# luanaruiz9/gated_gcrnns

Measured on AMD Instinct MI355X. Metric: sequences/sec (node), N=1000 K=5 T=32 F=64, higher is better.
Workload: dtype bf16

## Files before the change

gated_gcrnns_amd/_lib.py:

```python
import ctypes as C
import os

import torch

from . import build as _build

F32, F64, BF16 = 0, 1, 2

_c_i64 = C.c_int64
_c_p = C.c_void_p


class GcrnnError(RuntimeError):
    pass


def _load():
    path = os.environ.get('GCRNN_LIBPATH')
    if path:
        return _bind(C.CDLL(path))
    path = _build.LIBPATH
    if _build.needs_build() and os.path.exists(_build.HIPCC):
        _build.build(verbose=False)
    if not os.path.exists(path):
# ... 45 lines not shown
        'gcrnn_ell_assign_rows': (C.c_int, [_c_p, _c_p, _c_i64, _c_p, C.c_int, _c_i64, _c_p]),
        'gcrnn_fused_supported': (C.c_int, [_c_i64, _c_i64, _c_i64, _c_i64]),
        'gcrnn_fused_padded_nodes': (_c_i64, []),
        'gcrnn_fused_step_waves': (_c_i64, []),
        'gcrnn_fused_wgrad_waves': (_c_i64, []),
        'gcrnn_pack_seq_major': (C.c_int, [C.c_int, _c_p, _c_p, _c_i64, _c_i64, _c_i64, _c_i64, _c_i64, _c_p, _c_p]),
        'gcrnn_pack_seq_major_padded': (C.c_int, [_c_p, _c_p] + [_c_i64] * 6 + [_c_p]),
        'gcrnn_unpack_seq_major': (C.c_int, [C.c_int, _c_p, _c_p, _c_i64, _c_i64, _c_i64, _c_i64, _c_i64, _c_p, _c_p]),
        'gcrnn_fused_pack_weights': (C.c_int, [C.c_int, _c_p, _c_p, _c_p, _c_i64, _c_i64, _c_i64, _c_i64, _c_p]),
        'gcrnn_fused_forward_bf16': (C.c_int, [_c_p, _c_p, _c_p, _c_p, _c_p, _c_p, _c_p, _c_p, _c_p, _c_p, _c_p,
                                               _c_p, _c_p,
                                               _c_i64, _c_i64, _c_i64, _c_i64, _c_i64, _c_i64, _c_i64, _c_p, C.c_int, _c_p, C.c_double, _c_p, _c_p, _c_p, _c_p]),
        'gcrnn_fused_pack_weights_wide': (C.c_int, [C.c_int, _c_p, _c_p, _c_p, _c_i64, _c_i64, _c_i64, _c_i64, _c_i64, C.c_double, _c_p]),
        'gcrnn_fused_forward_wide_supported': (C.c_int, [_c_i64] * 7 + [C.c_double, C.c_int, C.c_int]),
        'gcrnn_fused_forward_wide_bf16': (C.c_int, [_c_p] * 10 + [_c_i64] * 7 + [_c_p, C.c_int, _c_p, _c_p, _c_p, _c_p]),
        'gcrnn_fused_backward_data_wide_supported': (C.c_int, [_c_i64] * 6 + [C.c_double, C.c_int, C.c_int]),
        'gcrnn_fused_backward_data_wide_bf16': (C.c_int, [_c_p] * 8 + [_c_i64] * 6 + [_c_p] * 7),
        'gcrnn_gate_readout_finish': (C.c_int, [_c_p, _c_i64, _c_p, _c_p, _c_p, _c_p, _c_i64, _c_p]),
        'gcrnn_fused_filter_output_wide_supported': (C.c_int, [_c_i64] * 7 + [C.c_double, C.c_int, C.c_int]),
        'gcrnn_fused_filter_output_wide_bf16': (C.c_int, [_c_p] * 7 + [_c_i64] * 7 + [_c_p, _c_p]),
        'gcrnn_fused_node_forward_wide_supported': (C.c_int, [_c_i64] * 6 + [C.c_double, C.c_int]),
        'gcrnn_fused_node_forward_wide_bf16': (C.c_int, [_c_p] * 11 + [_c_i64] * 6 + [_c_p, C.c_int, _c_p]),
        'gcrnn_fused_gate_pair_wide_supported': (C.c_int, [_c_i64] * 7 + [C.c_double, C.c_int, C.c_int]),
        'gcrnn_fused_gate_pair_prepass_wide_bf16': (C.c_int, [_c_p] * 12 + [_c_i64] * 7 + [_c_p, _c_p, _c_p, _c_p]),
        'gcrnn_fused_gate_pair_prepass_taps_wide_bf16': (C.c_int, [_c_p] * 7 + [_c_i64] + [_c_p] * 5 + [_c_i64] * 7 + [_c_p, _c_p, _c_p, _c_p]),
        'gcrnn_fused_inline_pack_supported': (C.c_int, [_c_i64, _c_i64, _c_i64, _c_i64, _c_i64, C.c_double]),
        'gcrnn_fused_seq_steps_per_launch': (_c_i64, [_c_i64] * 7 + [C.c_double, C.c_int, C.c_int, C.c_int]),
        'gcrnn_fused_filter_output_bf16': (C.c_int, [_c_p] * 11 + [_c_i64] * 7 + [C.c_double, C.c_int, _c_p]),
        'gcrnn_fused_node_forward_bf16': (C.c_int, [_c_p] * 15 + [_c_i64] * 6 + [_c_p, C.c_int, C.c_double, _c_p]),
        'gcrnn_fused_node_backward_data_bf16': (C.c_int, [_c_p] * 12 + [_c_i64] * 6 + [C.c_double, _c_p, C.c_int, _c_p]),
# ... 103 lines not shown
```

gated_gcrnns_amd/csrc/gcrnn_fused_seq32.h:

```cpp
#pragma once

#if defined(GCRNN_SEQ_STAMPS)
static __device__ unsigned long long gcrnn_seq32_stamps[256 * 96];
static __device__ __forceinline__ void gcrnn_stamp32_put(uint32_t lds_addr) {
  const unsigned long long tv = __builtin_amdgcn_s_memtime();
  asm volatile("ds_write_b64 %0, %1" ::"v"(lds_addr), "v"(tv) : "memory");
}
static __device__ __forceinline__ unsigned long long gcrnn_stamp32_get(uint32_t lds_addr) {
  unsigned long long tv;
  asm volatile("ds_read_b64 %0, %1\n\ts_waitcnt lgkmcnt(0)" : "=v"(tv) : "v"(lds_addr) : "memory");
  return tv;
}
#define GCRNN_STAMP32(slot)                                                                                   \
  do {                                                                                                        \
    if (wave == 0 && stamp_on && lane_now() == 0) gcrnn_stamp32_put((uint32_t)reinterpret_cast<uintptr_t>(smem) + M::FLAG_OFF + 8 * (slot)); \
  } while (0)
#define GCRNN_STAMP32_WAVE(slot0)                                                                             \
  do {                                                                                                        \
    if (stamp_on && lane_now() == 0) gcrnn_stamp32_put((uint32_t)reinterpret_cast<uintptr_t>(smem) + M::FLAG_OFF + 8 * ((slot0) + wave)); \
  } while (0)
#define GCRNN_STAMP32_FLUSH()                                                                                 \
  do {                                                                                                        \
    __syncthreads();                                                                                          \
    if (threadIdx.x < 96 && blockIdx.x < 256) gcrnn_seq32_stamps[blockIdx.x * 96 + threadIdx.x] = gcrnn_stamp32_get((uint32_t)reinterpret_cast<uintptr_t>(smem) + M::FLAG_OFF + 8 * threadIdx.x); \
// ... 63 lines not shown
  int hmod;
  const int32_t* flags;
  const float* gw;
  const uint4* tapf; float* taps_out; int ntaps;
  float* go;
  uint16_t* out1;
  const uint16_t* dh0_; int64_t dhstride;
  const uint16_t* hs0; int64_t hsstride;
  const float* gsc0; int64_t gscstride;
  float* gpart0; int64_t gpartstride;
  int final_raw;
  uint16_t* final_out; const uint16_t* final_h;
  const float* ng0; int64_t ngstride; int64_t nghalf;
  const float* r1a; const float* r1b;
  int stagger;
};

__device__ __forceinline__ int lane_now() {
  int ln;
  asm volatile("v_mbcnt_lo_u32_b32 %0, -1, 0\n\tv_mbcnt_hi_u32_b32 %0, -1, %0" : "=v"(ln));
  return ln;
}

#define GCRNN_HOP_ASM_WIDE32_STREAM(D)                                                             \
  do {                                                                                             \
    const int gwbeg = tbeg[0] >> 2, gwend = tend[STILES - 1] >> 2;                                 \
    if (gwbeg < gwend) {                                                                           \
      const int ls_ = lane_now(), r = ls_ & 15, q = ls_ >> 4;                                      \
      const uint32_t colb = lds_col + r * 8 + (q >> 1) * 4;        \
      const uint32_t qh_ = (uint32_t)(q & 1) << 4;                                                 \
// ... 22 lines not shown
  static_assert(16 * RS2 <= BIAS_OFF && FLAG_OFF + 768 <= WOFF, "LDS map");
  static size_t lds_bytes(int64_t entries, bool inline_pack, bool r1 = false) {
    const size_t need = (size_t)COL_OFF + (size_t)entries * 32 + GCRNN_HOP_COLUMN_PAD + NP * 4 + (r1 ? 2 * NP * 4 : 0) + (inline_pack ? (size_t)(32 * (XS > 0 ? XS : HS)) * NPCK * 2 : 0)
                        + PFS;
    return need <= 160 * 1024 ? need : 0;
  }
};

template <int K, int HS, int XS, int VAR, int MODE = 0, bool GATED = false, bool R1 = false, bool SPLIT = false>
__global__ __launch_bounds__(STHREADS) void fused_seq32_kernel(const Seq32Args a) {
  static_assert(!R1 || !SPLIT, "rank-1 graphs: every mode of the persistent form (the BPTT chain takes the adjoint plan: the factors swap)");
  static_assert(!SPLIT || ((MODE == 0 || MODE == 2) && !R1 && HS > 1), "split sequences: the (un-gated or time-gated) forward and the BPTT chain, with more than one chunk");
  constexpr bool ITEMS = (MODE == 1 || MODE == 3);
  constexpr bool SONLY = (MODE == 2 || MODE == 4);
  constexpr bool PKV = (VAR & 1) != 0, USERV = (VAR & 2) != 0 && (MODE == 0 || MODE == 4);
  static_assert(MODE == 0 || ((MODE >= 1 && MODE <= 4) && !GATED), "modes");
  static_assert(MODE < 3 || (!R1 && !SPLIT), "modes 3, 4: uniform-weight graphs, persistent form");
  using M = Seq32Map<K, HS, XS>;
  constexpr int KS = HS + XS;
  constexpr int F = 32 * HS, G = 32 * XS;
  constexpr int NCH = (MODE == 1) ? 2 * HS : HS;
  constexpr int PL = M::PL, WOFF = M::WOFF, WB = M::WB, COL_OFF = M::COL_OFF, RS2 = M::RS2;
  constexpr int NPCK = M::NPCK, NRND = NP / NPCK, NH = NCH * (K - 1), RPH = (NRND + NH - 1) / NH;
  constexpr int PKROWS = SONLY ? F : G;
  static_assert(STILES == 8 && GCRNN_HOP_ASM && K >= 2 && (SONLY ? XS == 0 : XS > 0), "generated hop stream: 8 tiles per wave; the chain's operand is the state alone");
  extern __shared__ __attribute__((aligned(16))) char smem[];
  const int entries = a.entries, B = a.B, N = a.N;

  const int tid = threadIdx.x, lane = tid & 63;
  const int wave = __builtin_amdgcn_readfirstlane(tid >> 6);
// ... 450 lines not shown
            lds_barrier();
            pack_drain(r0 + e);
          }
        }
#if !GCRNN_SEQ32_EP_FIRST
        if constexpr (SONLY && EPH > 0 && j <= EPH)
          ep_request(std::integral_constant<int, (j - 1) * STILES / (EPH > 0 ? EPH : 1)>{}, std::integral_constant<int, j * STILES / (EPH > 0 ? EPH : 1)>{});
#endif
        if (j < K - 1) lds_barrier();
        GCRNN_STAMP32(1 + chunk * 24 + 4 * (j - 1) + 4);
      };
      seq_static_for(hop, std::make_integer_sequence<int, K - 1>{});

      typedef __attribute__((__vector_size__(4 * sizeof(unsigned int)))) unsigned int u32x4_t;
      const int lane = lane_now(), q = lane >> 4, tl = wave * 64 + lane;
      auto request_next_operand = [&]() {
        if (ITEMS || !(last && more)) return;
        const int qo = lane_now() >> 4;
        int sw[STILES];
        slot_words(lane, sw);
        const __amdgpu_buffer_rsrc_t rsrc_hn = __builtin_amdgcn_make_buffer_rsrc(hout, 0, B * (NP * F * 2), 0x00020000);
#pragma unroll
        for (int s = 0; s < KS; ++s) {
          if (s == HS - 1) continue;
#pragma unroll
          for (int i = 0; i < STILES; ++i) {
            const int w = sw[i];
#ifdef GCRNN_SEQ32_EXPERIMENT_SKIP
            if ((GCRNN_SEQ32_EXPERIMENT_SKIP == 1) == (s < HS)) continue;
#endif
            if (s < HS)
              bfr[i][s] = __builtin_bit_cast(bf16x8, __builtin_amdgcn_raw_buffer_load_b128(rsrc_hn, (w >> 16) * (F * 2) + 16 * qo + 64 * s, b * (NP * F * 2), GCRNN_SEQ32_NT_XLOAD));
            else
              bfr[i][s] = __builtin_bit_cast(bf16x8, __builtin_amdgcn_raw_buffer_load_b128(rsrc_xn, (w >> 16) * (G * 2) + 16 * qo + 64 * (s - HS), b * (NP * G * 2), GCRNN_SEQ32_NT_XLOAD));
          }
        }
      };
      if (GCRNN_SEQ32_OPERAND_AT == 0) request_next_operand();
      if (ITEMS) GCRNN_STAMP32(1 + chunk * 24 + 19);
      float bs[2][4];
#pragma unroll
      for (int h = 0; h < 2; ++h)
#pragma unroll
        for (int e = 0; e < 4; ++e) bs[h][e] = (MODE >= 3 ? 1.f : (gin + gfo)) * lbias[chunk * 32 + q * 8 + h * 4 + e];
      u32x4_t pkd[STILES];
      int swe[STILES];
// ... 141 lines not shown
          if (lane == 0) gpart[(int64_t)b * (NCH * SWAVES) + chunk * SWAVES + wave] = part;
        }
      } else {
#pragma unroll
      for (int i = 0; i < STILES; ++i) {
        const int node = swe[i] >> 16;
        u32x4_t p{0u, 0u, 0u, 0u};
        if (node < N) {
          const f32x4 a0 = acc[i][0], a1 = acc[i][1];
          p[0] = pack2bf(fast_tanh(a0[0] + bs[0][0]), fast_tanh(a0[1] + bs[0][1]));
          p[1] = pack2bf(fast_tanh(a0[2] + bs[0][2]), fast_tanh(a0[3] + bs[0][3]));
          p[2] = pack2bf(fast_tanh(a1[0] + bs[1][0]), fast_tanh(a1[1] + bs[1][1]));
          p[3] = pack2bf(fast_tanh(a1[2] + bs[1][2]), fast_tanh(a1[3] + bs[1][3]));
        }
        pkd[i] = p;
        if (GCRNN_SEQ32_NT_STATE && last) __builtin_amdgcn_raw_buffer_store_b128(p, rsrc_o, node * (F * 2) + (chunk * 32 + q * 8) * 2, b * (NP * F * 2), GCRNN_SEQ32_NT_STATE);
        else __builtin_amdgcn_raw_buffer_store_b128(p, rsrc_o, node * (F * 2) + (chunk * 32 + q * 8) * 2, b * (NP * F * 2), 0);
        if (GCRNN_SEQ32_OPERAND_AT == 3 && last && more) {
          const __amdgpu_buffer_rsrc_t rsrc_hn = __builtin_amdgcn_make_buffer_rsrc(hout, 0, B * (NP * F * 2), 0x00020000);
#pragma unroll
          for (int s = 0; s < KS; ++s) {
            if (s == HS - 1) continue;
            if (s < HS)
              bfr[i][s] = __builtin_bit_cast(bf16x8, __builtin_amdgcn_raw_buffer_load_b128(rsrc_hn, node * (F * 2) + 16 * q + 64 * s, b * (NP * F * 2), 0));
            else
              bfr[i][s] = __builtin_bit_cast(bf16x8, __builtin_amdgcn_raw_buffer_load_b128(rsrc_xn, node * (G * 2) + 16 * q + 64 * (s - HS), b * (NP * G * 2), 0));
          }
        }
      }
      }
      GCRNN_STAMP32(1 + chunk * 24 + 17);
      if (!ITEMS && last) {
// ... 51 lines not shown
```

gated_gcrnns_amd/csrc/gcrnn_fused_seq32.hip:

```cpp
#include "gcrnn_fused_step.h"
#include "gcrnn_fused_seq32.h"

template <typename W>
__global__ void pack_weights_wide_kernel(const W* __restrict__ wA, const W* __restrict__ wB, uint16_t* __restrict__ out,
                                         int Fout, int F, int G, int Kin, int Kst, int K, float w) {
  const int KS = (F + G) / 32;
  const int64_t total = (int64_t)(Fout / 32) * K * 2 * KS * 64 * 8;
  const int64_t idx = (int64_t)blockIdx.x * blockDim.x + threadIdx.x;
  if (idx >= total) return;
  const int j = idx & 7, lane = (idx >> 3) & 63;
  int64_t rest = idx >> 9;
  const int s = rest % KS; rest /= KS;
  const int h = rest & 1; rest >>= 1;
  const int tap = rest % K;
  const int chunk = rest / K;
  const int m = lane & 15;
  const int f = chunk * 32 + 8 * (m >> 2) + 4 * h + (m & 3);
  const int feat = 32 * s + 8 * (lane >> 4) + j;
  float v = 0.f;
  if (feat < F) { if (tap < Kst) v = (float)wB[((int64_t)f * Kst + tap) * F + feat]; }
  else          { if (tap < Kin) v = (float)wA[((int64_t)f * Kin + tap) * G + (feat - F)]; }
  float sc = 1.f;
  for (int k = 0; k < tap; ++k) sc *= w;
  out[idx] = f2bf(v * sc);
// ... 158 lines not shown
    case 0: return seq32_launch_v<K, HS, XS, 0>(sa, lds, st);
    case 1: return seq32_launch_v<K, HS, XS, 1>(sa, lds, st);
    case 2: return seq32_launch_v<K, HS, XS, 2>(sa, lds, st);
    default: return seq32_launch_v<K, HS, XS, 3>(sa, lds, st);
  }
}

template <int K, int HS, int XS>
static int seq32_launch_pair(const Seq32Args& sa, bool inline_pack, hipStream_t st) {
  const size_t lds = seq32_lds<K, HS, XS>(sa.entries, inline_pack, sa.r1a != nullptr);
  if (!lds) return GCRNN_ERR_UNSUPPORTED;
  if (sa.r1a) return inline_pack ? seq32_launch_v<K, HS, XS, 1, 1, false, true>(sa, lds, st) : seq32_launch_v<K, HS, XS, 0, 1, false, true>(sa, lds, st);
  return inline_pack ? seq32_launch_v<K, HS, XS, 1, 1>(sa, lds, st) : seq32_launch_v<K, HS, XS, 0, 1>(sa, lds, st);
}

extern "C" int gcrnn_fused_forward_wide_bf16(const void* xs, const void* h0, void* hs, const void* wpack, const float* bias,
                                             const float* gi, const float* gf, const int32_t* tile_nodes, const int32_t* tile_off, const void* ell_col4, int64_t entries,
                                             int64_t B, int64_t T, int64_t N, int64_t F, int64_t G, int64_t K, void* Huser,
                                             int huser_last_only, const void* Xuser_inline, const float* rank1_a, const float* rank1_b,
                                             void* stream) {
  if (!xs || !h0 || !hs || !wpack || !tile_nodes || !tile_off || !ell_col4) return GCRNN_ERR_NULL_POINTER;
  if ((rank1_a == nullptr) != (rank1_b == nullptr)) return GCRNN_ERR_BAD_SHAPE;
  if ((gi == nullptr) != (gf == nullptr) || (gi && Xuser_inline)) return GCRNN_ERR_BAD_SHAPE;
  if (B <= 0 || T <= 0 || N <= 0 || N > NP || B > (1 << 24) || entries <= 0 || entries % 4) return GCRNN_ERR_BAD_SHAPE;
  if (B * (NP * (F > G ? F : G) * 2) > 2147483647LL || T * F * N > 2147483647LL) return GCRNN_ERR_BAD_SHAPE;
  if (Huser && (N % 8 != 0 || (reinterpret_cast<uintptr_t>(Huser) & 15))) return GCRNN_ERR_BAD_SHAPE;
  if (Xuser_inline && (N % 8 != 0 || (reinterpret_cast<uintptr_t>(Xuser_inline) & 15) || T * G * N > 2147483647LL)) return GCRNN_ERR_BAD_SHAPE;
  const int64_t xstep = B * NP * G, hstep = B * NP * F;
  Seq32Args sa{};
  sa.x0 = (const uint16_t*)xs; sa.xstride = xstep;
  sa.hfirst = (const uint16_t*)h0;
  sa.out0 = (uint16_t*)hs; sa.ostride = hstep;
  sa.wpack = (const uint4*)wpack; sa.bias = bias;
  sa.a1 = (const uint16_t*)Huser; sa.a1stride = F * N; sa.a1_last_only = huser_last_only ? 1 : 0;
  sa.ubstride = (int)((huser_last_only ? 1 : T) * F * N);
  sa.tile_nodes = tile_nodes; sa.tile_off = tile_off; sa.ell_col4 = (const uint2*)ell_col4;
  sa.entries = (int)entries; sa.B = (int)B; sa.N = (int)N;
  sa.nsteps = (int)T;
  sa.gi0 = gi; sa.gf0 = gf; sa.gstride = B;
  sa.r1a = rank1_a; sa.r1b = rank1_b;
  {
    const char* sg = getenv("GCRNN_SEQ32_STAGGER");
    sa.stagger = sg ? atoi(sg) : 0;
  }
  const bool inline_pack = Xuser_inline != nullptr && T > 2;
  if (inline_pack) {
    sa.pk_src0 = (const uint16_t*)Xuser_inline; sa.pksrc_stride = G * N;
    sa.pk_dst0 = const_cast<uint16_t*>(sa.x0); sa.pkdst_stride = xstep;
    sa.pk_stride = (int)(T * G * N);
  }
  hipStream_t st = as_stream(stream);
  const bool split = !rank1_a && !seq32_wanted(B) && seq32_split_wanted(B, F);
  const bool pack_split = Xuser_inline != nullptr && T > 1;
  if (split && pack_split && !inline_pack) {
    sa.pk_src0 = (const uint16_t*)Xuser_inline; sa.pksrc_stride = G * N;
    sa.pk_dst0 = const_cast<uint16_t*>(sa.x0); sa.pkdst_stride = xstep;
    sa.pk_stride = (int)(T * G * N);
  }
#define GCRNN_SEQ32_CASE(KK, HH, XX) if (K == KK && F == 32 * HH && G == 32 * XX) return seq32_launch<KK, HH, XX>(sa, split ? pack_split : inline_pack, st, split, T, N);
  GCRNN_SEQ32_CASE(5, 2, 2) GCRNN_SEQ32_CASE(4, 2, 2) GCRNN_SEQ32_CASE(3, 2, 2) GCRNN_SEQ32_CASE(2, 2, 2)
  GCRNN_SEQ32_CASE(5, 2, 1) GCRNN_SEQ32_CASE(4, 2, 1) GCRNN_SEQ32_CASE(3, 2, 1) GCRNN_SEQ32_CASE(2, 2, 1)
  GCRNN_SEQ32_CASE(5, 1, 1) GCRNN_SEQ32_CASE(4, 1, 1) GCRNN_SEQ32_CASE(3, 1, 1) GCRNN_SEQ32_CASE(2, 1, 1)
#undef GCRNN_SEQ32_CASE
  return GCRNN_ERR_UNSUPPORTED;
}


extern "C" int gcrnn_fused_gate_pair_wide_supported(int64_t B, int64_t T, int64_t N, int64_t F, int64_t G, int64_t K, int64_t entries,
                                                    double uniform_w, int img16, int with_pack) {
  if (uniform_w == 0.0 || !img16 || N <= 0 || N > NP || B <= 0 || T <= 0 || entries <= 0 || entries % 4) return 0;
  if (with_pack && (N % 8 || T * G * N > 2147483647LL)) return 0;
  if (B * T * (NP * (F > G ? F : G) * 2) > 2147483647LL) return 0;
  if (!seq32_wanted(B * T)) return 0;
  if (!seq32_lds_for(F, G, K, entries, with_pack != 0, (img16 & 2) != 0)) return 0;
  if (!with_pack) return 1;
  const int64_t first = B * T < gcrnn_persistent_grid() ? B * T : gcrnn_persistent_grid();
  return (int)((first + B - 1) / B);
}

// ... 177 lines not shown
```

gated_gcrnns_amd/ops.py:

```python
import ctypes as C
import os

import torch

from . import _lib
from ._lib import lib, check, dtype_code, GcrnnError


def _p(t):
    return C.c_void_p(t.data_ptr()) if t is not None else None


def _stream():
    return C.c_void_p(torch.cuda.current_stream().cuda_stream)


def require_device(*tensors):
    for t in tensors:
        if t is not None and not t.is_cuda:
            raise GcrnnError('gated_gcrnns_amd has no CPU path: move the module and its inputs to a ROCm '
                             'device (model.to("cuda"), x.cuda()); got a tensor on %s' % t.device)


def _pack_raw(x, perm=None):
# ... 296 lines not shown
    ok = fused_inline_pack_ok(plan, N, F, G, K)
    inline_arg = inline
    inline = (ok if inline is None else (ok and inline)) and X.data_ptr() % 16 == 0
    plan16 = fused_img16_plan(graph, False, None)
    wide = fused_wide_plan(graph, B, T, N, F, G, K, inline)
    if wide is None and plan16 is None:
        inl1 = inline_arg is not False and not os.environ.get('GCRNN_NO_INLINE_PACK') and X.data_ptr() % 16 == 0
        wide = fused_wide_plan(graph, B, T, N, F, G, K, inl1, rank1=True)
        if wide is None and inl1:
            inl1 = False
            wide = fused_wide_plan(graph, B, T, N, F, G, K, False, rank1=True)
        if wide is not None:
            inline = inl1
    if wide is not None:
        wpw = _fused_pack_weights_wide(wAc, wBc, wide['uniform_w'], st)
        for rep in range(reps + warm):
            if rep == warm:
                e0.record()
            _fused_forward_wide(wide, xs, h0s, hs, wAc, wBc, b32, B, T, N, F, G, K, H, False, Xc if inline else None, st, wpw=wpw)
        e1.record()
        torch.cuda.synchronize()
        per_step = 1e3 * e0.elapsed_time(e1) / (reps * T)
        return {'avg_us': per_step, 'launches': reps, 'inline_pack': bool(inline), 'steps_per_launch': T,
                'launch_avg_us': per_step * T, 'kernel': 'fused_seq32_kernel'}
    for rep in range(reps + 1):
        if rep == 1:
            torch.cuda.synchronize()
            e0.record()
        check(lib.gcrnn_fused_forward_bf16(_p(xs), _p(h0s), _p(hs), _p(wpack), _p(b32), None, None, *_fused_graph_args(plan16 or plan),
                                           B, T, N, F, G, K, _p(H) if H is not None else None, 2 if plan16 else 0, None, plan.get('uniform_w', 0.0),
                                           _p(Xc) if inline else None, None, None, st),
              'fused_forward')
    e1.record()
    torch.cuda.synchronize()
# ... 85 lines not shown
        return wpack
    return _cached_pack('taps32', (wA.detach(), wB.detach()), float(uniform_w), st, make)


def fused_wide_plan(graph, B, T, N, F, G, K, inline, rank1=False, gated=False):
    plan16 = fused_img16_plan(graph, False, None)
    if plan16 is None and rank1 and not os.environ.get('GCRNN_NO_IMG16'):
        plan16 = graph.fused_plan_rank1()
    if plan16 is None or F % 32 or G % 32:
        return None
    ok = lib.gcrnn_fused_forward_wide_supported(int(B), int(T), int(N), int(F), int(G), int(K), int(plan16['entries']),
                                                float(plan16.get('uniform_w', 0.0)), (3 if plan16.get('rank1') else 1) | (4 if gated else 0), 1 if inline else 0)
    return plan16 if ok else None


def _fused_forward_wide(plan16, xs, h0s, hs, wA, wB, b32, B, T, N, F, G, K, H, last_only, Xinline, st, wpw=None, gi=None, gf=None):
    if wpw is None:
        wpw = _fused_pack_weights_wide(wA.detach(), wB.detach(), plan16['uniform_w'], st)
    check(lib.gcrnn_fused_forward_wide_bf16(_p(xs), _p(h0s), _p(hs), _p(wpw), _p(b32), _p(gi), _p(gf), _p(plan16['tile_slots']), _p(plan16['tile_off']),
                                            _p(plan16['ell_col4']), plan16['entries'], B, T, N, F, G, K,
                                            _p(H) if H is not None else None, int(bool(last_only)), _p(Xinline) if Xinline is not None else None,
                                            _p(plan16.get('rank1_a')), _p(plan16.get('rank1_b')), st),
          'fused_forward_wide')


def fused_img16_plan(graph, gated, head):
    import os
    if os.environ.get('GCRNN_NO_IMG16'):
        return None
    return graph.fused_plan_img16()


def _fused_graph_args(plan):
# ... 11 lines not shown
    return s


def fused_inline_pack_ok(plan, N, F, G, K):
    if os.environ.get('GCRNN_NO_INLINE_PACK'):
        return False
    return bool(lib.gcrnn_fused_inline_pack_supported(int(N), int(F), int(G), int(K), int(plan['entries']), float(plan.get('uniform_w', 0.0))))


def fused_pad_taps(wA):
    F, G = wA.shape[0], wA.shape[3]
    Gp = fused_padded_inputs(F, G)
    return wA if Gp == G else torch.nn.functional.pad(wA, (0, Gp - G))


def fused_pack_inputs(X, h0, graph, overlap=False, first_only=False, channels=None):
    B, T, G, N = X.shape
    F = h0.shape[1]
    npad = graph.fused_plan()['npad']
    st = _stream()
    Xc, h0c = X.contiguous(), h0.contiguous()
    if channels is not None and channels != G:
        assert channels > G and not overlap and not first_only
        xs = torch.empty((T, B, npad, channels), dtype=torch.bfloat16, device=X.device)
        hs_all = torch.empty((T + 1, B, npad, F), dtype=torch.bfloat16, device=X.device)
        check(lib.gcrnn_pack_seq_major(_lib.BF16, _p(h0c), _p(hs_all), B, 1, F, N, npad, None, st), 'pack_seq')
        check(lib.gcrnn_pack_seq_major_padded(_p(Xc), _p(xs), B, T, G, channels, N, npad, st), 'pack_seq_padded')
        return xs, hs_all
    xs = torch.empty((T, B, npad, G), dtype=torch.bfloat16, device=X.device)
    hs_all = torch.empty((T + 1, B, npad, F), dtype=torch.bfloat16, device=X.device)
    check(lib.gcrnn_pack_seq_major(_lib.BF16, _p(h0c), _p(hs_all), B, 1, F, N, npad, None, st), 'pack_seq')
    if first_only:
        check(lib.gcrnn_pack_seq_major_steps(_p(Xc), _p(xs), B, T, G, N, npad, 0, min(2, T), 0, st), 'pack_seq_steps')
        return xs, hs_all
    if not overlap:
        check(lib.gcrnn_pack_seq_major(_lib.BF16, _p(Xc), _p(xs), B, T, G, N, npad, None, st), 'pack_seq')
        return xs, hs_all
    main = torch.cuda.current_stream(X.device)
    side = _side_stream(X.device)
    check(lib.gcrnn_pack_seq_major_steps(_p(Xc), _p(xs), B, T, G, N, npad, 0, 1, 0, st), 'pack_seq_steps')
    ready = torch.cuda.Event()
    ready.record(main)
    side.wait_event(ready)
    events = [None] * T
    sst = C.c_void_p(side.cuda_stream)
    blocks = int(os.environ.get('GCRNN_PACK_BLOCKS', torch.cuda.get_device_properties(X.device).multi_processor_count))
    for t in range(1, T):
        check(lib.gcrnn_pack_seq_major_steps(_p(Xc), _p(xs), B, T, G, N, npad, t, t + 1, blocks, sst), 'pack_seq_steps')
        ev = torch.cuda.Event()
        ev.record(side)
        events[t] = ev
    Xc.record_stream(side)
    xs.record_stream(side)
    return xs, hs_all, events


def fused_pack_inputs_gated(X, h0, graph, F, K):
    B, T, G, N = X.shape
    plan = graph.fused_plan()
    plan16 = fused_img16_plan(graph, True, None)
    steps = 0
    if plan16 is not None and X.dtype == torch.bfloat16 and X.is_contiguous() and X.data_ptr() % 16 == 0 and not os.environ.get('GCRNN_NO_INLINE_PACK'):
        _, steps = fused_gate_pair_plan(graph, B, T, N, F, G, K, True)
        if steps <= 0:
            steps = int(lib.gcrnn_fused_gate_prepass_lays_out(B, T, N, F, G, K, plan16['entries'], plan.get('uniform_w', 0.0), 1))
    if steps <= 0 or steps >= T:
        return fused_pack_inputs(X, h0, graph)
    npad = plan['npad']
    st = _stream()
    xs = torch.empty((T, B, npad, G), dtype=torch.bfloat16, device=X.device)
    hs_all = torch.empty((T + 1, B, npad, F), dtype=torch.bfloat16, device=X.device)
    check(lib.gcrnn_pack_seq_major(_lib.BF16, _p(h0.contiguous()), _p(hs_all), B, 1, F, N, npad, None, st), 'pack_seq')
    check(lib.gcrnn_pack_seq_major_steps(_p(X), _p(xs), B, T, G, N, npad, 0, steps, 0, st), 'pack_seq_steps')
    xs._pending_user = X
    xs._pending_steps = steps
    return xs, hs_all


def _pending_layout_for(xs, consumer_steps):
    x_user = getattr(xs, '_pending_user', None)
    if x_user is None:
        return None
    done = int(getattr(xs, '_pending_steps', 0))
    if consumer_steps > 0 and consumer_steps == done:
        return x_user
    T, B, npad, G = xs.shape
# ... 109 lines not shown
            Xz[:, :, :X.shape[2]] = X
            X = Xz
    elif packed is None:
        X, wA = fused_pad_operands(X, wA.detach())
    B, T, _, N = X.shape
    G = wA.shape[3]
    F = wA.shape[0]
    K = max(wA.shape[2], wB.shape[2])
    plan = graph.fused_plan()
    st = _stream()
    dev = X.device
    X = X.contiguous()
    h0 = h0.contiguous()
    events = None
    inline = False
    if packed is not None:
        xs, hs_all = packed
    elif gates is None and gate_values is None and X.data_ptr() % 16 == 0 and (
            fused_inline_pack_ok(plan, N, F, G, K) or (head is None and not os.environ.get('GCRNN_NO_INLINE_PACK')
                                                       and fused_wide_plan(graph, B, T, N, F, G, K, True, rank1=True) is not None)):
        xs, hs_all = fused_pack_inputs(X, h0, graph, first_only=True)
        inline = True
    elif gates is None and fused_overlap_ok(X):
        xs, hs_all, events = fused_pack_inputs(X, h0, graph, overlap=True)
    elif gates is not None and gate_values is None:
        xs, hs_all = fused_pack_inputs_gated(X, h0, graph, F, K)
    else:
        xs, hs_all = fused_pack_inputs(X, h0, graph)
    h0s, hs = hs_all[:1], hs_all[1:]
    gi = gf = None
    if gate_values is not None:
        gi, gf = (g.detach().float().contiguous() for g in gate_values)
        assert tuple(gi.shape) == (T, B) and tuple(gf.shape) == (T, B)
    elif gates is not None:
        hzero = fused_h0_zero_flag(h0)
        g = {}
        gp = {}
        for name in ('in', 'forget'):
            wA_g, wB_g, bias_g, lin_w, lin_b = gates[name]
            if wA_g.shape[3] != G:
                wA_g = torch.nn.functional.pad(wA_g.detach(), (0, G - wA_g.shape[3]))
            assert max(wA_g.shape[2], wB_g.shape[2]) == K and wA_g.shape[0] == F
            gp[name] = (wA_g, wB_g, bias_g, lin_w, lin_b)
# ... 20 lines not shown
        check(lib.gcrnn_fused_forward_bf16(_p(xs), _p(h0s), _p(hs), _p(wpack), _p(b32), _p(gi), _p(gf), *_fused_graph_args(plan16 or plan),
                                           B, T, N, F, G, K, None, 2 if plan16 else 0, evs, plan.get('uniform_w', 0.0), _p(X) if inline else None,
                                           _p(hw), _p(part), st), 'fused_forward')
        y = part.sum(dim=2)
        if head[1] is not None:
            y = y + head[1].detach().float().reshape(())
        return y.permute(1, 0, 2).unsqueeze(2).contiguous()
    wide = fused_wide_plan(graph, B, T, N, F, G, K, inline, rank1=True, gated=(gi is not None)) if (evs is None and head is None and not (gi is not None and inline)) else None
    if wide is not None:
        if native_out:
            assert not return_states
            _fused_forward_wide(wide, xs, h0s, hs, wA, wB, b32, B, T, N, F, G, K, None, False, X if inline else None, st, gi=gi, gf=gf)
            Hv = hs.permute(1, 0, 3, 2)[:, :, :, :N]
            return Hv[:, T - 1:] if last_only else Hv
        H = torch.empty((B, 1 if last_only else T, F, N), dtype=torch.bfloat16, device=dev)
        _fused_forward_wide(wide, xs, h0s, hs, wA, wB, b32, B, T, N, F, G, K, H if direct else None, last_only, X if inline else None, st, gi=gi, gf=gf)
        if not direct:
            src = hs[T - 1:] if last_only else hs
            check(lib.gcrnn_unpack_seq_major(_lib.BF16, _p(src), _p(H), B, 1 if last_only else T, F, N, plan['npad'], None, st), 'unpack_seq')
        if return_states:
            return hs_all, plan, H
        return H
    plan16 = fused_img16_plan(graph, gi is not None, None)
    wpack = _fused_pack_weights(wA, wB, st)
    if native_out:
        assert not return_states
        check(lib.gcrnn_fused_forward_bf16(_p(xs), _p(h0s), _p(hs), _p(wpack), _p(b32), _p(gi), _p(gf), *_fused_graph_args(plan16 or plan),
                                           B, T, N, F, G, K, None, (2 if plan16 else 0), evs,
                                           plan.get('uniform_w', 0.0), _p(X) if inline else None, None, None, st),
              'fused_forward')
        Hv = hs.permute(1, 0, 3, 2)[:, :, :, :N]
        return Hv[:, T - 1:] if last_only else Hv
    H = torch.empty((B, 1 if last_only else T, F, N), dtype=torch.bfloat16, device=dev)
    check(lib.gcrnn_fused_forward_bf16(_p(xs), _p(h0s), _p(hs), _p(wpack), _p(b32), _p(gi), _p(gf), *_fused_graph_args(plan16 or plan),
                                       B, T, N, F, G, K, _p(H) if direct else None, int(last_only) | (2 if plan16 else 0), evs,
                                       plan.get('uniform_w', 0.0), _p(X) if inline else None, None, None, st),
          'fused_forward')
# ... 2147 lines not shown
```

include/gcrnn.h:

```cpp
#ifndef GCRNN_H
#define GCRNN_H

#include <stdint.h>

#ifdef __cplusplus
extern "C" {
#endif

enum { GCRNN_F32 = 0, GCRNN_F64 = 1, GCRNN_BF16 = 2 };

enum {
  GCRNN_OK = 0,
  GCRNN_ERR_BAD_DTYPE = 1,
  GCRNN_ERR_BAD_SHAPE = 2,
  GCRNN_ERR_NULL_POINTER = 3,
  GCRNN_ERR_UNSUPPORTED = 4,
  GCRNN_ERR_LAUNCH = 5,
  GCRNN_ERR_WORKSPACE = 6
};

int gcrnn_version(void);
const char* gcrnn_status_string(int status);
const char* gcrnn_last_hip_error(void);

// ... 162 lines not shown
                             const void* Xuser_inline ,
                             const float* head_w ,
                             float* head_part ,
                             void* stream);

int gcrnn_fused_pack_weights_wide(int wdtype, const void* wA, const void* wB, void* wpack, int64_t Fout, int64_t F, int64_t G, int64_t Kin,
                                  int64_t Kst, double uniform_w, void* stream);
int gcrnn_fused_forward_wide_supported(int64_t B, int64_t T, int64_t N, int64_t F, int64_t G, int64_t K, int64_t entries, double uniform_w,
                                       int img16, int inline_pack);
int gcrnn_fused_forward_wide_bf16(const void* xs, const void* h0, void* hs, const void* wpack, const float* bias, const float* gi,
                                  const float* gf, const int32_t* tile_nodes, const int32_t* tile_off, const void* ell_col4, int64_t entries,
                                  int64_t B, int64_t T, int64_t N, int64_t F, int64_t G, int64_t K, void* Huser, int huser_last_only,
                                  const void* Xuser_inline,
                                  const float* rank1_a, const float* rank1_b ,
                                  void* stream);
int gcrnn_fused_gate_pair_wide_supported(int64_t B, int64_t T, int64_t N, int64_t F, int64_t G, int64_t K, int64_t entries, double uniform_w,
                                         int img16, int with_pack);
int gcrnn_fused_backward_data_wide_supported(int64_t B, int64_t T, int64_t N, int64_t F, int64_t K, int64_t entries, double uniform_w, int img16,
                                             int inline_pack);
int gcrnn_fused_backward_data_wide_bf16(const void* dHs, const void* hs, void* dpre, void* dh0, const void* wpackT, const int32_t* tile_nodes,
                                        const int32_t* tile_off, const void* ell_col4, int64_t entries, int64_t B, int64_t T, int64_t N,
                                        int64_t F, int64_t K, const float* gf, const void* h0s, float* dgf_parts, const void* dHuser_inline,
                                        const float* rank1_a, const float* rank1_b, void* stream);
int gcrnn_fused_filter_output_wide_supported(int64_t B, int64_t T, int64_t N, int64_t F, int64_t G, int64_t K, int64_t entries, double uniform_w,
                                             int img16, int with_pack );
int gcrnn_fused_filter_output_wide_bf16(const void* xs, const void* wpack, const float* bias, void* out, const int32_t* tile_nodes,
                                        const int32_t* tile_off, const void* ell_col4, int64_t entries, int64_t B, int64_t T, int64_t N,
                                        int64_t F, int64_t G, int64_t K,
                                        const void* x_user ,
                                        void* stream);
// ... 173 lines not shown
```

Before: 148,100.

## Route persistent forward hidden state through per-workgroup scratch instead of full state image

Adds a scratch-buffer variant of the persistent wide forward kernel. When no states are returned, the hidden state for non-final channel chunks is stored to and reloaded from a small per-workgroup scratch region, rather than written to the full T×B×NP×F sequence-major state image. The Python side also stops allocating the T-step state image on this lean path. This is meant to cut global memory traffic and allocation size. In exchange it adds a new kernel variant and a buffer sized by grid and channel count, and it falls back when the split form is selected.

```diff
diff --git a/gated_gcrnns_amd/_lib.py b/gated_gcrnns_amd/_lib.py
--- a/gated_gcrnns_amd/_lib.py
+++ b/gated_gcrnns_amd/_lib.py
@@ -83,6 +83,8 @@
         'gcrnn_fused_pack_weights_wide': (C.c_int, [C.c_int, _c_p, _c_p, _c_p, _c_i64, _c_i64, _c_i64, _c_i64, _c_i64, C.c_double, _c_p]),
         'gcrnn_fused_forward_wide_supported': (C.c_int, [_c_i64] * 7 + [C.c_double, C.c_int, C.c_int]),
         'gcrnn_fused_forward_wide_bf16': (C.c_int, [_c_p] * 10 + [_c_i64] * 7 + [_c_p, C.c_int, _c_p, _c_p, _c_p, _c_p]),
+        'gcrnn_fused_forward_wide_scratch_bytes': (_c_i64, [_c_i64, _c_i64, C.c_int]),
+        'gcrnn_fused_forward_wide_scratch_bf16': (C.c_int, [_c_p] * 3 + [_c_i64] + [_c_p] * 7 + [_c_i64] * 7 + [_c_p, C.c_int, _c_p, _c_p, _c_p, _c_p]),
         'gcrnn_fused_backward_data_wide_supported': (C.c_int, [_c_i64] * 6 + [C.c_double, C.c_int, C.c_int]),
         'gcrnn_fused_backward_data_wide_bf16': (C.c_int, [_c_p] * 8 + [_c_i64] * 6 + [_c_p] * 7),
         'gcrnn_gate_readout_finish': (C.c_int, [_c_p, _c_i64, _c_p, _c_p, _c_p, _c_p, _c_i64, _c_p]),
diff --git a/gated_gcrnns_amd/csrc/gcrnn_fused_seq32.h b/gated_gcrnns_amd/csrc/gcrnn_fused_seq32.h
--- a/gated_gcrnns_amd/csrc/gcrnn_fused_seq32.h
+++ b/gated_gcrnns_amd/csrc/gcrnn_fused_seq32.h
@@ -101,6 +101,7 @@
   const float* ng0; int64_t ngstride; int64_t nghalf;
   const float* r1a; const float* r1b;
   int stagger;
+  uint16_t* scr;
 };
 
 __device__ __forceinline__ int lane_now() {
@@ -153,6 +154,9 @@
   constexpr bool ITEMS = (MODE == 1 || MODE == 3);
   constexpr bool SONLY = (MODE == 2 || MODE == 4);
   constexpr bool PKV = (VAR & 1) != 0, USERV = (VAR & 2) != 0 && (MODE == 0 || MODE == 4);
+  constexpr bool SCRV = (VAR & 4) != 0;
+  static_assert(!SCRV || (MODE == 0 && !SPLIT && (VAR & 2) != 0), "state scratch: the persistent forward with the user-layout output");
+  constexpr int SCR_CH = NP * 64;
   static_assert(MODE == 0 || ((MODE >= 1 && MODE <= 4) && !GATED), "modes");
   static_assert(MODE < 3 || (!R1 && !SPLIT), "modes 3, 4: uniform-weight graphs, persistent form");
   using M = Seq32Map<K, HS, XS>;
@@ -633,12 +637,16 @@
 
       typedef __attribute__((__vector_size__(4 * sizeof(unsigned int)))) unsigned int u32x4_t;
       const int lane = lane_now(), q = lane >> 4, tl = wave * 64 + lane;
+      auto scratch_rsrc = [&]() {
+        return __builtin_amdgcn_make_buffer_rsrc(SCRV ? a.scr + (int64_t)blockIdx.x * ((HS - 1) * (SCR_CH / 2)) : nullptr, 0, SCRV ? (HS - 1) * SCR_CH : 0, 0x00020000);
+      };
       auto request_next_operand = [&]() {
         if (ITEMS || !(last && more)) return;
         const int qo = lane_now() >> 4;
         int sw[STILES];
         slot_words(lane, sw);
-        const __amdgpu_buffer_rsrc_t rsrc_hn = __builtin_amdgcn_make_buffer_rsrc(hout, 0, B * (NP * F * 2), 0x00020000);
+        const __amdgpu_buffer_rsrc_t rsrc_hn = __builtin_amdgcn_make_buffer_rsrc(SCRV ? nullptr : hout, 0, SCRV ? 0 : B * (NP * F * 2), 0x00020000);
+        [[maybe_unused]] const __amdgpu_buffer_rsrc_t rsrc_sn = scratch_rsrc();
 #pragma unroll
         for (int s = 0; s < KS; ++s) {
           if (s == HS - 1) continue;
@@ -648,7 +656,9 @@
 #ifdef GCRNN_SEQ32_EXPERIMENT_SKIP
             if ((GCRNN_SEQ32_EXPERIMENT_SKIP == 1) == (s < HS)) continue;
 #endif
-            if (s < HS)
+            if (SCRV && s < HS)
+              bfr[i][s] = __builtin_bit_cast(bf16x8, __builtin_amdgcn_raw_buffer_load_b128(rsrc_sn, (lane_now() & 15) * 64 + 16 * qo, s * SCR_CH + (wave * STILES + i) * 1024, 16));
+            else if (s < HS)
               bfr[i][s] = __builtin_bit_cast(bf16x8, __builtin_amdgcn_raw_buffer_load_b128(rsrc_hn, (w >> 16) * (F * 2) + 16 * qo + 64 * s, b * (NP * F * 2), GCRNN_SEQ32_NT_XLOAD));
             else
               bfr[i][s] = __builtin_bit_cast(bf16x8, __builtin_amdgcn_raw_buffer_load_b128(rsrc_xn, (w >> 16) * (G * 2) + 16 * qo + 64 * (s - HS), b * (NP * G * 2), GCRNN_SEQ32_NT_XLOAD));
@@ -820,8 +830,12 @@
           p[3] = pack2bf(fast_tanh(a1[2] + bs[1][2]), fast_tanh(a1[3] + bs[1][3]));
         }
         pkd[i] = p;
+        if constexpr (SCRV) {
+          if (!last) __builtin_amdgcn_raw_buffer_store_b128(p, scratch_rsrc(), (lane & 15) * 64 + 16 * q, chunk * SCR_CH + (wave * STILES + i) * 1024, 0);
+        } else
         if (GCRNN_SEQ32_NT_STATE && last) __builtin_amdgcn_raw_buffer_store_b128(p, rsrc_o, node * (F * 2) + (chunk * 32 + q * 8) * 2, b * (NP * F * 2), GCRNN_SEQ32_NT_STATE);
         else __builtin_amdgcn_raw_buffer_store_b128(p, rsrc_o, node * (F * 2) + (chunk * 32 + q * 8) * 2, b * (NP * F * 2), 0);
+        static_assert(!SCRV || GCRNN_SEQ32_OPERAND_AT != 3, "state scratch: the per-tile request form reads the state image");
         if (GCRNN_SEQ32_OPERAND_AT == 3 && last && more) {
           const __amdgpu_buffer_rsrc_t rsrc_hn = __builtin_amdgcn_make_buffer_rsrc(hout, 0, B * (NP * F * 2), 0x00020000);
 #pragma unroll
diff --git a/gated_gcrnns_amd/csrc/gcrnn_fused_seq32.hip b/gated_gcrnns_amd/csrc/gcrnn_fused_seq32.hip
--- a/gated_gcrnns_amd/csrc/gcrnn_fused_seq32.hip
+++ b/gated_gcrnns_amd/csrc/gcrnn_fused_seq32.hip
@@ -196,23 +196,47 @@
   return inline_pack ? seq32_launch_v<K, HS, XS, 1, 1>(sa, lds, st) : seq32_launch_v<K, HS, XS, 0, 1>(sa, lds, st);
 }
 
-extern "C" int gcrnn_fused_forward_wide_bf16(const void* xs, const void* h0, void* hs, const void* wpack, const float* bias,
-                                             const float* gi, const float* gf, const int32_t* tile_nodes, const int32_t* tile_off, const void* ell_col4, int64_t entries,
-                                             int64_t B, int64_t T, int64_t N, int64_t F, int64_t G, int64_t K, void* Huser,
-                                             int huser_last_only, const void* Xuser_inline, const float* rank1_a, const float* rank1_b,
-                                             void* stream) {
-  if (!xs || !h0 || !hs || !wpack || !tile_nodes || !tile_off || !ell_col4) return GCRNN_ERR_NULL_POINTER;
+int gcrnn_seq32s_forward(const Seq32Args& sa, int K, int HS, int XS, bool inline_pack, size_t lds, hipStream_t st);
+
+static int64_t seq32_scratch_need(int64_t B, int64_t F) {
+  const int64_t wgs = B < gcrnn_persistent_grid() ? B : gcrnn_persistent_grid();
+  return wgs * (F / 32 - 1) * (int64_t)NP * 64;
+}
+
+extern "C" int64_t gcrnn_fused_forward_wide_scratch_bytes(int64_t B, int64_t F, int rank1) {
+  if (B <= 0 || F <= 0 || F % 32) return -1;
+  const char* sw = getenv("GCRNN_SEQ32_STATE_SCRATCH");
+  if (sw && sw[0] == '0') return -1;
+  const char* p32 = getenv("GCRNN_SEQ32P");
+  if (p32 && p32[0] != '0') return -1;
+  if (!rank1 && !seq32_wanted(B) && seq32_split_wanted(B, F)) return -1;
+  return seq32_scratch_need(B, F);
+}
+
+static int forward_wide_impl(const void* xs, const void* h0, void* hs, void* scratch, int64_t scratch_bytes, bool no_image, const void* wpack, const float* bias,
+                             const float* gi, const float* gf, const int32_t* tile_nodes, const int32_t* tile_off, const void* ell_col4, int64_t entries,
+                             int64_t B, int64_t T, int64_t N, int64_t F, int64_t G, int64_t K, void* Huser,
+                             int huser_last_only, const void* Xuser_inline, const float* rank1_a, const float* rank1_b,
+                             void* stream) {
+  if (!xs || !h0 || (!no_image && !hs) || !wpack || !tile_nodes || !tile_off || !ell_col4) return GCRNN_ERR_NULL_POINTER;
+  if (no_image && !Huser) return GCRNN_ERR_NULL_POINTER;
   if ((rank1_a == nullptr) != (rank1_b == nullptr)) return GCRNN_ERR_BAD_SHAPE;
   if ((gi == nullptr) != (gf == nullptr) || (gi && Xuser_inline)) return GCRNN_ERR_BAD_SHAPE;
   if (B <= 0 || T <= 0 || N <= 0 || N > NP || B > (1 << 24) || entries <= 0 || entries % 4) return GCRNN_ERR_BAD_SHAPE;
   if (B * (NP * (F > G ? F : G) * 2) > 2147483647LL || T * F * N > 2147483647LL) return GCRNN_ERR_BAD_SHAPE;
   if (Huser && (N % 8 != 0 || (reinterpret_cast<uintptr_t>(Huser) & 15))) return GCRNN_ERR_BAD_SHAPE;
   if (Xuser_inline && (N % 8 != 0 || (reinterpret_cast<uintptr_t>(Xuser_inline) & 15) || T * G * N > 2147483647LL)) return GCRNN_ERR_BAD_SHAPE;
+  if (no_image) {
+    if (F % 32 || F < 32) return GCRNN_ERR_UNSUPPORTED;
+    const int64_t need = seq32_scratch_need(B, F);
+    if (scratch_bytes < need || (need > 0 && (!scratch || (reinterpret_cast<uintptr_t>(scratch) & 15)))) return GCRNN_ERR_BAD_SHAPE;
+  }
   const int64_t xstep = B * NP * G, hstep = B * NP * F;
   Seq32Args sa{};
   sa.x0 = (const uint16_t*)xs; sa.xstride = xstep;
   sa.hfirst = (const uint16_t*)h0;
-  sa.out0 = (uint16_t*)hs; sa.ostride = hstep;
+  sa.out0 = no_image ? nullptr : (uint16_t*)hs; sa.ostride = hstep;
+  sa.scr = no_image ? (uint16_t*)scratch : nullptr;
   sa.wpack = (const uint4*)wpack; sa.bias = bias;
   sa.a1 = (const uint16_t*)Huser; sa.a1stride = F * N; sa.a1_last_only = huser_last_only ? 1 : 0;
   sa.ubstride = (int)((huser_last_only ? 1 : T) * F * N);
@@ -233,6 +257,19 @@
   }
   hipStream_t st = as_stream(stream);
   const bool split = !rank1_a && !seq32_wanted(B) && seq32_split_wanted(B, F);
+  if (no_image) {
+    if (split) return GCRNN_ERR_UNSUPPORTED;
+#define GCRNN_SEQ32_CASE(KK, HH, XX) \
+    if (K == KK && F == 32 * HH && G == 32 * XX) { \
+      const size_t lds = seq32_lds<KK, HH, XX>(sa.entries, inline_pack, sa.r1a != nullptr); \
+      return lds ? gcrnn_seq32s_forward(sa, KK, HH, XX, inline_pack, lds, st) : GCRNN_ERR_UNSUPPORTED; \
+    }
+    GCRNN_SEQ32_CASE(5, 2, 2) GCRNN_SEQ32_CASE(4, 2, 2) GCRNN_SEQ32_CASE(3, 2, 2) GCRNN_SEQ32_CASE(2, 2, 2)
+    GCRNN_SEQ32_CASE(5, 2, 1) GCRNN_SEQ32_CASE(4, 2, 1) GCRNN_SEQ32_CASE(3, 2, 1) GCRNN_SEQ32_CASE(2, 2, 1)
+    GCRNN_SEQ32_CASE(5, 1, 1) GCRNN_SEQ32_CASE(4, 1, 1) GCRNN_SEQ32_CASE(3, 1, 1) GCRNN_SEQ32_CASE(2, 1, 1)
+#undef GCRNN_SEQ32_CASE
+    return GCRNN_ERR_UNSUPPORTED;
+  }
   const bool pack_split = Xuser_inline != nullptr && T > 1;
   if (split && pack_split && !inline_pack) {
     sa.pk_src0 = (const uint16_t*)Xuser_inline; sa.pksrc_stride = G * N;
@@ -245,6 +282,24 @@
   GCRNN_SEQ32_CASE(5, 1, 1) GCRNN_SEQ32_CASE(4, 1, 1) GCRNN_SEQ32_CASE(3, 1, 1) GCRNN_SEQ32_CASE(2, 1, 1)
 #undef GCRNN_SEQ32_CASE
   return GCRNN_ERR_UNSUPPORTED;
+}
+
+extern "C" int gcrnn_fused_forward_wide_bf16(const void* xs, const void* h0, void* hs, const void* wpack, const float* bias,
+                                             const float* gi, const float* gf, const int32_t* tile_nodes, const int32_t* tile_off, const void* ell_col4, int64_t entries,
+                                             int64_t B, int64_t T, int64_t N, int64_t F, int64_t G, int64_t K, void* Huser,
+                                             int huser_last_only, const void* Xuser_inline, const float* rank1_a, const float* rank1_b,
+                                             void* stream) {
+  return forward_wide_impl(xs, h0, hs, nullptr, 0, false, wpack, bias, gi, gf, tile_nodes, tile_off, ell_col4, entries, B, T, N, F, G, K, Huser,
+                           huser_last_only, Xuser_inline, rank1_a, rank1_b, stream);
+}
+
+extern "C" int gcrnn_fused_forward_wide_scratch_bf16(const void* xs, const void* h0, void* scratch, int64_t scratch_bytes, const void* wpack, const float* bias,
+                                                     const float* gi, const float* gf, const int32_t* tile_nodes, const int32_t* tile_off, const void* ell_col4,
+                                                     int64_t entries, int64_t B, int64_t T, int64_t N, int64_t F, int64_t G, int64_t K, void* Huser,
+                                                     int huser_last_only, const void* Xuser_inline, const float* rank1_a, const float* rank1_b,
+                                                     void* stream) {
+  return forward_wide_impl(xs, h0, nullptr, scratch, scratch_bytes, true, wpack, bias, gi, gf, tile_nodes, tile_off, ell_col4, entries, B, T, N, F, G, K, Huser,
+                           huser_last_only, Xuser_inline, rank1_a, rank1_b, stream);
 }
 
 
diff --git a/gated_gcrnns_amd/csrc/gcrnn_fused_seq32s.hip b/gated_gcrnns_amd/csrc/gcrnn_fused_seq32s.hip
--- /dev/null
+++ b/gated_gcrnns_amd/csrc/gcrnn_fused_seq32s.hip
@@ -0,0 +1,35 @@
+#include "gcrnn_fused_step.h"
+#define GCRNN_SEQ32_STAMP_READER_NAME gcrnn_debug_read_seq32s_stamps
+#include "gcrnn_fused_seq32.h"
+
+template <int K, int HS, int XS, int VAR, bool GATED, bool R1>
+static int seq32s_launch_v(const Seq32Args& sa, size_t lds, hipStream_t st) {
+  static_assert((VAR & 6) == 6, "state scratch: with the user-layout output");
+  auto sk = fused_seq32_kernel<K, HS, XS, VAR, 0, GATED, R1>;
+  if (hipFuncSetAttribute(reinterpret_cast<const void*>(sk), hipFuncAttributeMaxDynamicSharedMemorySize, (int)lds) != hipSuccess)
+    return GCRNN_ERR_LAUNCH;
+  GCRNN_PRE_LAUNCH();
+  sk<<<(unsigned)(sa.B < gcrnn_persistent_grid() ? sa.B : gcrnn_persistent_grid()), STHREADS, lds, st>>>(sa);
+  GCRNN_CHECK_LAUNCH();
+  return GCRNN_OK;
+}
+
+template <int K, int HS, int XS>
+static int seq32s_launch(const Seq32Args& sa, bool inline_pack, size_t lds, hipStream_t st) {
+  if (!sa.a1 || (HS > 1 && !sa.scr)) return GCRNN_ERR_NULL_POINTER;
+  if (sa.gi0) {
+    if (inline_pack) return GCRNN_ERR_BAD_SHAPE;
+    return sa.r1a ? seq32s_launch_v<K, HS, XS, 6, true, true>(sa, lds, st) : seq32s_launch_v<K, HS, XS, 6, true, false>(sa, lds, st);
+  }
+  if (sa.r1a) return inline_pack ? seq32s_launch_v<K, HS, XS, 7, false, true>(sa, lds, st) : seq32s_launch_v<K, HS, XS, 6, false, true>(sa, lds, st);
+  return inline_pack ? seq32s_launch_v<K, HS, XS, 7, false, false>(sa, lds, st) : seq32s_launch_v<K, HS, XS, 6, false, false>(sa, lds, st);
+}
+
+int gcrnn_seq32s_forward(const Seq32Args& sa, int K, int HS, int XS, bool inline_pack, size_t lds, hipStream_t st) {
+#define GCRNN_SEQ32S_CASE(KK, HH, XX) if (K == KK && HS == HH && XS == XX) return seq32s_launch<KK, HH, XX>(sa, inline_pack, lds, st);
+  GCRNN_SEQ32S_CASE(5, 2, 2) GCRNN_SEQ32S_CASE(4, 2, 2) GCRNN_SEQ32S_CASE(3, 2, 2) GCRNN_SEQ32S_CASE(2, 2, 2)
+  GCRNN_SEQ32S_CASE(5, 2, 1) GCRNN_SEQ32S_CASE(4, 2, 1) GCRNN_SEQ32S_CASE(3, 2, 1) GCRNN_SEQ32S_CASE(2, 2, 1)
+  GCRNN_SEQ32S_CASE(5, 1, 1) GCRNN_SEQ32S_CASE(4, 1, 1) GCRNN_SEQ32S_CASE(3, 1, 1) GCRNN_SEQ32S_CASE(2, 1, 1)
+#undef GCRNN_SEQ32S_CASE
+  return GCRNN_ERR_UNSUPPORTED;
+}
diff --git a/gated_gcrnns_amd/ops.py b/gated_gcrnns_amd/ops.py
--- a/gated_gcrnns_amd/ops.py
+++ b/gated_gcrnns_amd/ops.py
@@ -334,10 +334,11 @@
             inline = inl1
     if wide is not None:
         wpw = _fused_pack_weights_wide(wAc, wBc, wide['uniform_w'], st)
+        scr = fused_state_scratch(wide, B, F, dev) if H is not None else None
         for rep in range(reps + warm):
             if rep == warm:
                 e0.record()
-            _fused_forward_wide(wide, xs, h0s, hs, wAc, wBc, b32, B, T, N, F, G, K, H, False, Xc if inline else None, st, wpw=wpw)
+            _fused_forward_wide(wide, xs, h0s, hs, wAc, wBc, b32, B, T, N, F, G, K, H, False, Xc if inline else None, st, wpw=wpw, scratch=scr)
         e1.record()
         torch.cuda.synchronize()
         per_step = 1e3 * e0.elapsed_time(e1) / (reps * T)
@@ -453,9 +454,24 @@
     return plan16 if ok else None
 
 
-def _fused_forward_wide(plan16, xs, h0s, hs, wA, wB, b32, B, T, N, F, G, K, H, last_only, Xinline, st, wpw=None, gi=None, gf=None):
+def fused_state_scratch(plan16, B, F, dev):
+    need = int(lib.gcrnn_fused_forward_wide_scratch_bytes(int(B), int(F), 1 if plan16.get('rank1') else 0))
+    if need < 0:
+        return None
+    return torch.empty((need,), dtype=torch.uint8, device=dev)
+
+
+def _fused_forward_wide(plan16, xs, h0s, hs, wA, wB, b32, B, T, N, F, G, K, H, last_only, Xinline, st, wpw=None, gi=None, gf=None, scratch=None):
     if wpw is None:
         wpw = _fused_pack_weights_wide(wA.detach(), wB.detach(), plan16['uniform_w'], st)
+    if scratch is not None:
+        assert H is not None
+        check(lib.gcrnn_fused_forward_wide_scratch_bf16(_p(xs), _p(h0s), _p(scratch), int(scratch.numel()), _p(wpw), _p(b32), _p(gi), _p(gf), _p(plan16['tile_slots']),
+                                                        _p(plan16['tile_off']), _p(plan16['ell_col4']), plan16['entries'], B, T, N, F, G, K,
+                                                        _p(H), int(bool(last_only)), _p(Xinline) if Xinline is not None else None,
+                                                        _p(plan16.get('rank1_a')), _p(plan16.get('rank1_b')), st),
+              'fused_forward_wide_scratch')
+        return
     check(lib.gcrnn_fused_forward_wide_bf16(_p(xs), _p(h0s), _p(hs), _p(wpw), _p(b32), _p(gi), _p(gf), _p(plan16['tile_slots']), _p(plan16['tile_off']),
                                             _p(plan16['ell_col4']), plan16['entries'], B, T, N, F, G, K,
                                             _p(H) if H is not None else None, int(bool(last_only)), _p(Xinline) if Xinline is not None else None,
@@ -497,21 +513,22 @@
     return wA if Gp == G else torch.nn.functional.pad(wA, (0, Gp - G))
 
 
-def fused_pack_inputs(X, h0, graph, overlap=False, first_only=False, channels=None):
+def fused_pack_inputs(X, h0, graph, overlap=False, first_only=False, channels=None, states=True):
     B, T, G, N = X.shape
     F = h0.shape[1]
     npad = graph.fused_plan()['npad']
     st = _stream()
+    TS = T if states else 0
     Xc, h0c = X.contiguous(), h0.contiguous()
     if channels is not None and channels != G:
         assert channels > G and not overlap and not first_only
         xs = torch.empty((T, B, npad, channels), dtype=torch.bfloat16, device=X.device)
-        hs_all = torch.empty((T + 1, B, npad, F), dtype=torch.bfloat16, device=X.device)
+        hs_all = torch.empty((TS + 1, B, npad, F), dtype=torch.bfloat16, device=X.device)
         check(lib.gcrnn_pack_seq_major(_lib.BF16, _p(h0c), _p(hs_all), B, 1, F, N, npad, None, st), 'pack_seq')
         check(lib.gcrnn_pack_seq_major_padded(_p(Xc), _p(xs), B, T, G, channels, N, npad, st), 'pack_seq_padded')
         return xs, hs_all
     xs = torch.empty((T, B, npad, G), dtype=torch.bfloat16, device=X.device)
-    hs_all = torch.empty((T + 1, B, npad, F), dtype=torch.bfloat16, device=X.device)
+    hs_all = torch.empty((TS + 1, B, npad, F), dtype=torch.bfloat16, device=X.device)
     check(lib.gcrnn_pack_seq_major(_lib.BF16, _p(h0c), _p(hs_all), B, 1, F, N, npad, None, st), 'pack_seq')
     if first_only:
         check(lib.gcrnn_pack_seq_major_steps(_p(Xc), _p(xs), B, T, G, N, npad, 0, min(2, T), 0, st), 'pack_seq_steps')
@@ -538,7 +555,7 @@
     return xs, hs_all, events
 
 
-def fused_pack_inputs_gated(X, h0, graph, F, K):
+def fused_pack_inputs_gated(X, h0, graph, F, K, states=True):
     B, T, G, N = X.shape
     plan = graph.fused_plan()
     plan16 = fused_img16_plan(graph, True, None)
@@ -548,11 +565,11 @@
         if steps <= 0:
             steps = int(lib.gcrnn_fused_gate_prepass_lays_out(B, T, N, F, G, K, plan16['entries'], plan.get('uniform_w', 0.0), 1))
     if steps <= 0 or steps >= T:
-        return fused_pack_inputs(X, h0, graph)
+        return fused_pack_inputs(X, h0, graph, states=states)
     npad = plan['npad']
     st = _stream()
     xs = torch.empty((T, B, npad, G), dtype=torch.bfloat16, device=X.device)
-    hs_all = torch.empty((T + 1, B, npad, F), dtype=torch.bfloat16, device=X.device)
+    hs_all = torch.empty(((T if states else 0) + 1, B, npad, F), dtype=torch.bfloat16, device=X.device)
     check(lib.gcrnn_pack_seq_major(_lib.BF16, _p(h0.contiguous()), _p(hs_all), B, 1, F, N, npad, None, st), 'pack_seq')
     check(lib.gcrnn_pack_seq_major_steps(_p(X), _p(xs), B, T, G, N, npad, 0, steps, 0, st), 'pack_seq_steps')
     xs._pending_user = X
@@ -692,19 +709,20 @@
     h0 = h0.contiguous()
     events = None
     inline = False
+    lean = packed is None and head is None and not return_states and not native_out and N % 8 == 0
     if packed is not None:
         xs, hs_all = packed
     elif gates is None and gate_values is None and X.data_ptr() % 16 == 0 and (
             fused_inline_pack_ok(plan, N, F, G, K) or (head is None and not os.environ.get('GCRNN_NO_INLINE_PACK')
                                                        and fused_wide_plan(graph, B, T, N, F, G, K, True, rank1=True) is not None)):
-        xs, hs_all = fused_pack_inputs(X, h0, graph, first_only=True)
+        xs, hs_all = fused_pack_inputs(X, h0, graph, first_only=True, states=not lean)
         inline = True
     elif gates is None and fused_overlap_ok(X):
-        xs, hs_all, events = fused_pack_inputs(X, h0, graph, overlap=True)
+        xs, hs_all, events = fused_pack_inputs(X, h0, graph, overlap=True, states=not lean)
     elif gates is not None and gate_values is None:
-        xs, hs_all = fused_pack_inputs_gated(X, h0, graph, F, K)
+        xs, hs_all = fused_pack_inputs_gated(X, h0, graph, F, K, states=not lean)
     else:
-        xs, hs_all = fused_pack_inputs(X, h0, graph)
+        xs, hs_all = fused_pack_inputs(X, h0, graph, states=not lean)
     h0s, hs = hs_all[:1], hs_all[1:]
     gi = gf = None
     if gate_values is not None:
@@ -755,13 +773,18 @@
             Hv = hs.permute(1, 0, 3, 2)[:, :, :, :N]
             return Hv[:, T - 1:] if last_only else Hv
         H = torch.empty((B, 1 if last_only else T, F, N), dtype=torch.bfloat16, device=dev)
-        _fused_forward_wide(wide, xs, h0s, hs, wA, wB, b32, B, T, N, F, G, K, H if direct else None, last_only, X if inline else None, st, gi=gi, gf=gf)
+        scr = fused_state_scratch(wide, B, F, dev) if (direct and not return_states) else None
+        if scr is None and hs.shape[0] == 0:
+            hs = torch.empty((T,) + tuple(h0s.shape[1:]), dtype=torch.bfloat16, device=dev)
+        _fused_forward_wide(wide, xs, h0s, hs, wA, wB, b32, B, T, N, F, G, K, H if direct else None, last_only, X if inline else None, st, gi=gi, gf=gf, scratch=scr)
         if not direct:
             src = hs[T - 1:] if last_only else hs
             check(lib.gcrnn_unpack_seq_major(_lib.BF16, _p(src), _p(H), B, 1 if last_only else T, F, N, plan['npad'], None, st), 'unpack_seq')
         if return_states:
             return hs_all, plan, H
         return H
+    if hs.shape[0] == 0:
+        hs = torch.empty((T,) + tuple(h0s.shape[1:]), dtype=torch.bfloat16, device=dev)
     plan16 = fused_img16_plan(graph, gi is not None, None)
     wpack = _fused_pack_weights(wA, wB, st)
     if native_out:
diff --git a/include/gcrnn.h b/include/gcrnn.h
--- a/include/gcrnn.h
+++ b/include/gcrnn.h
@@ -200,6 +200,12 @@
                                   const void* Xuser_inline,
                                   const float* rank1_a, const float* rank1_b ,
                                   void* stream);
+int64_t gcrnn_fused_forward_wide_scratch_bytes(int64_t B, int64_t F, int rank1);
+int gcrnn_fused_forward_wide_scratch_bf16(const void* xs, const void* h0, void* scratch, int64_t scratch_bytes, const void* wpack,
+                                          const float* bias, const float* gi, const float* gf, const int32_t* tile_nodes,
+                                          const int32_t* tile_off, const void* ell_col4, int64_t entries, int64_t B, int64_t T, int64_t N,
+                                          int64_t F, int64_t G, int64_t K, void* Huser, int huser_last_only, const void* Xuser_inline,
+                                          const float* rank1_a, const float* rank1_b, void* stream);
 int gcrnn_fused_gate_pair_wide_supported(int64_t B, int64_t T, int64_t N, int64_t F, int64_t G, int64_t K, int64_t entries, double uniform_w,
                                          int img16, int with_pack);
 int gcrnn_fused_backward_data_wide_supported(int64_t B, int64_t T, int64_t N, int64_t F, int64_t K, int64_t entries, double uniform_w, int img16,
```

Measured after the change: 160,400, median of 6. 1.08x the previous value.
